# qingpingmo/OCN

Measured on AMD Instinct MI355X. Metric: candidate-edges/sec (CN predictor fwd), ogbl-collab shape, higher is better.
Workload: dtype f32

## Files before the change

### include/ocn_hip.h

```cpp
#ifndef OCN_HIP_H
#define OCN_HIP_H

#include <stdint.h>

#ifdef __cplusplus
extern "C" {
#endif

#define OCN_ABI_VERSION 9
#define OCN_EINVAL (-1)
#define OCN_ECAP   (-2)

#define OCN_ST_CAP  1
#define OCN_ST_SCAN 2
#define OCN_SCAN_POISON (-1)

#define OCN_F_CN1 1u
#define OCN_F_CN2 2u

int ocn_abi_version(void);

int64_t ocn_scan_workspace_bytes(int64_t n);

int ocn_zero_regions(void* const* ptrs, const int64_t* bytes, int32_t n, void* stream);
// ... 125 lines not shown
                          int64_t n_cols, const int64_t* rows, int64_t Q, int32_t drop_self,
                          int64_t window_cols , const int64_t* off ,
                          int64_t* edges , void* stream);
int32_t ocn_segment_topk_max_k(void);
int ocn_segment_topk(const float* scores, const int64_t* ptr, int64_t Q, int32_t k, float* top_val, int64_t* top_pos,
                     void* stream);

int ocn_philox4x32(const uint32_t* ctr , uint32_t key0, uint32_t key1, int64_t n, uint32_t* out ,
                   void* stream);
int ocn_complement_count(const int64_t* rowptrK, const int32_t* colK, int64_t n_cols, int32_t* count ,
                         void* stream);
int32_t ocn_sample_stage_cols(void);
int ocn_sample_complement_rows(const int64_t* rowptrK, const int32_t* colK, int64_t n_cols, const int64_t* rows, int64_t Q,
                               int64_t per, int64_t q0, uint64_t seed, int64_t* out , void* stream);
int ocn_sample_complement_pairs(const int64_t* rowptrK, const int32_t* colK, int64_t n_cols,
                                const int64_t* cptr , int64_t T, int64_t t0, uint64_t seed,
                                int64_t* out , void* stream);

int ocn_gather_schedule(const int32_t* gcost, int64_t n_groups, int64_t segment, int32_t* perm, void* stream);

int ocn_cn_weights_cn6(uint64_t* histA, uint64_t* histB, int64_t N, const float* innerprod, int32_t* scalars,
                       float* nip_out, const float* s2_exact , const float* s3_exact ,
                       void* stream);
int ocn_cn_gather3(const int64_t* rowptrA, const int32_t* colA, const int64_t* src, const int64_t* dst,
                   const int64_t* order, int64_t B, const int64_t* off, const uint8_t* flagsA,
                   const uint8_t* flagsB, const float* weightsA, const float* weightsB, const float* nip,
                   const float* h, int32_t H, float* xcn1, float* xcn2, float* xcn3, float* xij, void* stream);

int ocn_cn3_flags(const int64_t* rowptrA, const int32_t* colA, const int64_t* rowptrT, const int32_t* colT,
                  const uint32_t* bitmapP, int64_t bm_stride_words, const int64_t* src, const int64_t* dst,
                  const int64_t* order , int64_t B, int64_t n_cols, const int64_t* off, uint8_t* flags,
                  int64_t flags_cap, uint64_t* hist , int32_t* cnt3, int32_t* status,
                  const int64_t* nds , const int64_t* chunk_off , void* stream);

int ocn_cn_gather3_backward(const int64_t* rowptrA, const int32_t* colA, const int64_t* src, const int64_t* dst,
                            const int64_t* order, int64_t B, const int64_t* off, const uint8_t* flagsA,
                            const uint8_t* flagsB, const float* weightsA, const float* weightsB, const float* nip,
                            const float* h, int32_t H, const float* g1, const float* g2, const float* g3,
                            const float* g4, float* dh, void* stream);

int ocn_cn_gather_backward(const int64_t* rowptrA, const int32_t* colA,
                           const int64_t* src, const int64_t* dst, const int64_t* order, int64_t B,
                           const int64_t* off, const uint8_t* flags, const int32_t* wc,
                           const float* weights, const float* h, int32_t H,
                           const float* g1, const float* g2, const float* g3, float* dh, void* stream);

int64_t ocn_cn_gather_backward_det_workspace_bytes(int64_t N, int64_t B, int64_t flags_cap);
int ocn_cn_gather_backward_det(const int64_t* rowptrA, const int32_t* colA, const int64_t* src, const int64_t* dst,
                               int64_t B, const int64_t* off, const uint8_t* flags, const int32_t* wc, int64_t flags_cap,
                               const float* weights, const float* h, int64_t N, int32_t H, const float* g1,
                               const float* g2, const float* g3, float* dh, void* workspace, void* stream);
int64_t ocn_cn_gather_backward_det_keys_offset(int64_t N);
int ocn_cn_gather_backward_det_lists(const int64_t* rowptrA, const int32_t* colA, const int64_t* src, const int64_t* dst,
                                     int64_t B, const int64_t* off, const uint8_t* flags, int64_t flags_cap, int64_t N,
                                     void* workspace, void* stream);

int ocn_spmm_csr(const int64_t* rowptr, const int32_t* col, const float* val, int64_t n_rows,
                 const float* x, int32_t F, const float* pre, const float* post,
                 int32_t mode, int32_t edge_scale, int32_t self_mode,
                 float* y, void* stream);

int ocn_spmm_csr_rows(const int64_t* rowptr, const int32_t* col, const float* val, int64_t n_rows,
                      const float* x, int32_t F, const float* pre, const float* post,
                      int32_t mode, int32_t edge_scale, int32_t self_mode,
                      const int64_t* rows, int64_t n_list, float* y, void* stream);

int ocn_spmm_csr_max_arg(const int64_t* rowptr, const int32_t* col, const float* val, int64_t n_rows,
                         const float* x, int32_t F, float* y, int32_t* arg, void* stream);
int ocn_spmm_max_backward(const int64_t* rowptrT, const int32_t* colT, const float* valT, int64_t n_rows,
                          const int32_t* arg, const float* g, int32_t F, float* gx, void* stream);

int ocn_deg_rsqrt(const int64_t* rowptr, const float* val, int64_t n_rows, float add, float* out,
                  void* stream);

int64_t ocn_spgemm_max_cols(void);
int ocn_spgemm_pattern_count(const int64_t* rowptrA, const int32_t* colA, int64_t n_rows,
                             const int64_t* rowptrB, const int32_t* colB, int64_t n_colsB,
                             int32_t* row_count, uint32_t* bitmap ,
                             int64_t bm_stride_words, void* stream);
int ocn_spgemm_pattern_fill(const int64_t* rowptrA, const int32_t* colA, int64_t n_rows,
                            const int64_t* rowptrB, const int32_t* colB, int64_t n_colsB,
                            const int64_t* rowptrC, int32_t* colC, void* stream);
int32_t ocn_cn_flags_small_graph_cols(void);
int ocn_spgemm_bit_rows(const int64_t* rowptrA, const int32_t* colA, int64_t n_rows, const int64_t* rowptrB, const int32_t* colB,
                        int64_t n_colsB, const int64_t* rows, int64_t n_req, int32_t* done, uint32_t* bitmap,
                        int64_t bm_stride_words, void* stream);

int ocn_dense_from_csr(const int64_t* rowptr, const int32_t* col, int64_t n, int64_t ld, int8_t* dense, int8_t* denseT,
                       void* stream);
int ocn_dense_block_mm_bits(const int8_t* A, const int8_t* Bt, int64_t ld, int64_t K, int32_t r0, int32_t r1, int32_t c0,
                            int32_t c1, int32_t fold, uint32_t* bits, int64_t bm_stride_words, void* stream);
int ocn_bitrows_from_csr(const int64_t* rowptr, const int32_t* col, int64_t n_rows, uint32_t* bits, int64_t bm_stride_words,
                         void* stream);
int ocn_bitrows_count(const uint32_t* bits, int64_t bm_stride_words, int64_t n_rows, int64_t n_cols, int32_t* row_count,
                      void* stream);
int ocn_bitrows_fill(const uint32_t* bits, int64_t bm_stride_words, int64_t n_rows, int64_t n_cols, const int64_t* rowptr,
                     int32_t* col, void* stream);

int ocn_csr_union_count(const int64_t* rowptrA, const int32_t* colA, const int64_t* rowptrB, const int32_t* colB,
                        int64_t n_rows, int32_t* count, void* stream);
int ocn_csr_union_fill(const int64_t* rowptrA, const int32_t* colA, const int64_t* rowptrB, const int32_t* colB,
                       int64_t n_rows, const int64_t* rowptrC , int32_t* colC, void* stream);
int64_t ocn_bitrows_insert_workspace_bytes(int64_t nnzD);
int ocn_bitrows_insert(const int64_t* rowptrA, const int32_t* colA, const int64_t* rowptrT, const int32_t* colT,
                       const int64_t* rowptrD, const int32_t* colD, int64_t n, int64_t nnzD, uint32_t* bits,
                       int64_t bm_stride_words, int32_t* added, void* workspace, void* stream);

int ocn_csr_minus_count(const int64_t* rowptrA, const int32_t* colA, const int64_t* rowptrB, const int32_t* colB,
                        int64_t n_rows, int32_t* count, void* stream);
int ocn_csr_minus_fill(const int64_t* rowptrA, const int32_t* colA, const int64_t* rowptrB, const int32_t* colB,
                       int64_t n_rows, const int64_t* rowptrC , int32_t* colC, void* stream);
int64_t ocn_bitrows_remove_workspace_bytes(int64_t nnzD);
int ocn_bitrows_remove(const int64_t* rowptrA0, const int32_t* colA0, const int64_t* rowptrT0, const int32_t* colT0,
                       const int64_t* rowptrA, const int32_t* colA, const int64_t* rowptrT, const int32_t* colT,
                       const int64_t* rowptrD, const int32_t* colD, int64_t n, int64_t nnzD, uint32_t* bits,
                       int64_t bm_stride_words, int32_t* removed, void* workspace, void* stream);

int64_t ocn_rows_neighbourhood_workspace_bytes(int64_t n_list);
int ocn_rows_neighbourhood(const int64_t* rowptrT, const int32_t* colT, int64_t n, const int64_t* rows, int64_t n_list,
                           uint32_t* bits, void* workspace, void* stream);
int ocn_bitlist_count(const uint32_t* bits, int64_t n_bits, int32_t* count, void* stream);
int ocn_bitlist_fill(const uint32_t* bits, int64_t n_bits, const int64_t* off , int64_t* out,
                     void* stream);

int ocn_rows_ln_relu(const float* x, const float* gamma, const float* beta, float eps, int32_t relu,
                     int64_t rows, int32_t H, float* y, void* stream);
int ocn_combine3(const float* coef, const float* x1, const float* x2, const float* x3, int64_t n,
                 float* out, void* stream);

int ocn_fill_rows(float* dst, int64_t ld, int32_t n_cols, const float* vec, const int64_t* row_range,
                  int64_t max_rows, void* stream);

typedef struct OcnLinearGroup {
  const float* X; int64_t ldX;
  int64_t M;
  const void* Wp;
  const float* bias;
  const float* gamma; const float* beta; float eps;
  int32_t relu;
  const float* scale;
  const float* addend; int64_t ldAdd;
  const float* dotw; const float* dotb;
  float* Y; int64_t ldY;
  const int64_t* row_range;
  const int64_t* y_row_map;
  int32_t add_bcast;
} OcnLinearGroup;

int64_t ocn_linear_panel_bytes(int32_t N, int32_t K);
int ocn_linear_split_weight(const float* W, int32_t N, int32_t K, void* Wp, void* stream);
int ocn_linear_bf16x6(const float* X, int64_t M, int32_t K, const void* Wp, int32_t N,
                      const float* bias, const float* gamma, const float* beta, float eps,
                      int32_t relu, const float* dotw, const float* dotb, float* Y, void* stream);
int ocn_linear_grouped(const OcnLinearGroup* groups, int32_t n_groups, int32_t K, int32_t N, void* stream);

typedef struct OcnHeadsArgs {
  const float* x[3];
  int64_t ldx, B;
  int32_t H;
  const void* p_first[3];
  const void* p_mid[2];
  const void* p_out[3];
  const float* vec;
  const int64_t* ranges;
  const int64_t* y_row_map;
  float* y;
// ... 42 lines not shown
```

### ocn_amd/_lib.py

```python
from __future__ import annotations

import ctypes
import glob
import os
import subprocess
from ctypes import c_float, c_int32, c_int64, c_void_p

_HERE = os.path.dirname(os.path.abspath(__file__))
_ROOT = os.path.dirname(_HERE)
LIB_PATH = os.environ.get("OCN_LIB_PATH", os.path.join(_HERE, "libocn_hip.so"))
CSRC = os.path.join(_HERE, "csrc")
INCLUDE = os.path.join(_ROOT, "include")

_P = c_void_p
ABI_VERSION = 9
SIGNATURES = {
    "ocn_abi_version": (c_int32, []),
    "ocn_scan_workspace_bytes": (c_int64, [c_int64]),
    "ocn_zero_regions": (c_int32, [_P, _P, c_int32, _P]),
    "ocn_check_edges": (c_int32, [_P, _P, c_int64, c_int64, c_int64, _P, _P]),
    "ocn_edge_offsets": (c_int32, [_P, _P, c_int64, _P, _P, _P]),
    "ocn_class_order": (c_int32, [_P, _P, _P, c_int64, _P, _P, _P, _P, _P, _P]),
    "ocn_scan_i32": (c_int32, [_P, c_int64, _P, _P, _P]),
    "ocn_order_workspace_bytes": (c_int64, [c_int64]),
    "ocn_order_by_node": (c_int32, [_P, c_int64, c_int64, _P, _P, _P]),
    "ocn_order_by_node_finish": (c_int32, [_P, c_int64, c_int64, _P, _P, _P]),
    "ocn_order_by_node_finish_rec": (c_int32, [_P, _P, _P, _P, c_int64, c_int64, _P, _P, _P, _P]),
    "ocn_batch_prep": (c_int32, [_P, _P, c_int64, _P, _P, c_int64, _P, _P, _P, c_int32, _P]),
    "ocn_cn_flags": (c_int32, [_P, _P, _P, _P, _P, _P, _P, c_int64, _P, c_int64, _P, _P, _P, c_int64, c_int64, _P, _P, c_int64, _P,
                               _P, _P, _P, _P, _P, _P]),
    "ocn_cn_flags_rec": (c_int32, [_P, _P, _P, _P, _P, _P, _P, c_int64, _P, c_int64, _P, _P, _P, c_int64, c_int64, _P, _P, c_int64, _P,
                                   _P, _P, _P, _P, _P, _P]),
    "ocn_chunk_offsets": (c_int32, [_P, _P, _P, _P, c_int64, _P, _P, _P]),
    "ocn_walk_chunk": (c_int32, []),
    "ocn_cn_walk_flags": (c_int32, [_P, _P, _P, _P, _P, _P, c_int64, _P, _P, _P, c_int64, _P, _P, c_int64, _P, _P, _P,
                                    _P, _P]),
    "ocn_neighbor_degree_sum": (c_int32, [_P, _P, c_int64, _P, _P]),
    "ocn_walk_prep_max_batch": (c_int32, []),
    "ocn_cn_flags_small_graph_cols": (c_int32, []),
    "ocn_walk_prep": (c_int32, [_P, _P, _P, _P, c_int64, c_int32, _P, _P, _P, _P, _P, _P, _P, _P, _P, _P, _P, _P, _P]),
    "ocn_cn_walk_group": (c_int32, [_P, _P, _P, _P, _P, c_int64, _P, _P, _P, _P, _P, _P, _P, c_int64, _P, _P, _P, _P]),
    "ocn_walk_rev_offsets": (c_int32, [_P, _P, _P, _P, _P, c_int64, _P, _P, _P]),
    "ocn_cn_weights_cn5": (c_int32, [_P, c_int64, _P, _P, c_int32, _P, _P]),
    "ocn_cn5_column_stats": (c_int32, [_P, c_int64, _P, _P]),
    "ocn_cn_colsum_workspace_bytes": (c_int64, [c_int64, c_int64]),
    "ocn_cn_colsum_exact": (c_int32, [_P, _P, _P, c_int64, _P, _P, _P, _P, c_int64, _P, c_int64, _P, _P, _P, _P, _P, _P, _P]),
    "ocn_cn_weights_cn7": (c_int32, [_P, c_int64, c_float, _P, _P, _P]),
    "ocn_cn_gather": (c_int32, [_P, _P, _P, _P, _P, c_int64, _P, _P, _P, _P, _P, c_int32, c_int64, _P, _P, _P, _P, _P,
                                _P, _P, _P, _P, _P]),
    "ocn_cn8_pool": (c_int32, [_P, _P, _P, _P, _P, _P, _P, c_int64, _P, c_int64, _P, _P, _P, c_int64, c_int64, _P, c_int32, _P, _P,
                               _P, _P, _P, _P]),
    "ocn_cn_node_sums": (c_int32, [_P, _P, _P, _P, _P, _P, _P, c_int64, _P, c_int64, _P, _P, _P, c_int64, c_int64, _P, _P, _P, _P, _P,
                                   _P, _P]),
    "ocn_row_diff_stage_cols": (c_int32, []),
    "ocn_row_diff_count": (c_int32, [_P, _P, _P, _P, _P, c_int64, c_int32, _P, _P]),
    "ocn_row_diff_fill": (c_int32, [_P, _P, _P, _P, _P, c_int64, c_int32, _P, _P, _P]),
    "ocn_two_hop_window_cols": (c_int64, []),
    "ocn_two_hop_diff_count": (c_int32, [_P, _P, _P, _P, c_int64, _P, c_int64, c_int32, c_int64, _P, _P]),
    "ocn_two_hop_diff_fill": (c_int32, [_P, _P, _P, _P, c_int64, _P, c_int64, c_int32, c_int64, _P, _P, _P]),
    "ocn_segment_topk_max_k": (c_int32, []),
    "ocn_segment_topk": (c_int32, [_P, _P, c_int64, c_int32, _P, _P, _P]),
    "ocn_philox4x32": (c_int32, [_P, ctypes.c_uint32, ctypes.c_uint32, c_int64, _P, _P]),
    "ocn_complement_count": (c_int32, [_P, _P, c_int64, _P, _P]),
    "ocn_sample_stage_cols": (c_int32, []),
    "ocn_sample_complement_rows": (c_int32, [_P, _P, c_int64, _P, c_int64, c_int64, c_int64, ctypes.c_uint64, _P, _P]),
    "ocn_sample_complement_pairs": (c_int32, [_P, _P, c_int64, _P, c_int64, c_int64, ctypes.c_uint64, _P, _P]),
    "ocn_gather_schedule": (c_int32, [_P, c_int64, c_int64, _P, _P]),
    "ocn_coo_to_csr_workspace_bytes": (c_int64, [c_int64, c_int64, c_int32, c_int32]),
    "ocn_coo_to_csr": (c_int32, [_P, _P, c_int64, c_int64, c_int64, c_int32, c_int32, _P, _P, _P, _P, _P]),
    "ocn_wgrad_workspace_bytes": (c_int64, [c_int64, c_int32, c_int32]),
    "ocn_wgrad": (c_int32, [_P, c_int64, _P, c_int64, c_int64, c_int32, c_int32, _P, _P, _P, _P]),
    "ocn_cn_weights_cn6": (c_int32, [_P, _P, c_int64, _P, _P, _P, _P, _P, _P]),
    "ocn_cn_gather3": (c_int32, [_P, _P, _P, _P, _P, c_int64, _P, _P, _P, _P, _P, _P, _P, c_int32, _P, _P, _P, _P, _P]),
    "ocn_cn3_flags": (c_int32, [_P, _P, _P, _P, _P, c_int64, _P, _P, _P, c_int64, c_int64, _P, _P, c_int64, _P, _P, _P, _P, _P, _P]),
    "ocn_cn_gather3_backward": (c_int32, [_P, _P, _P, _P, _P, c_int64, _P, _P, _P, _P, _P, _P, _P, c_int32, _P, _P, _P, _P, _P, _P]),
    "ocn_cn_gather_backward": (c_int32, [_P, _P, _P, _P, _P, c_int64, _P, _P, _P, _P, _P, c_int32, _P, _P, _P, _P, _P]),
    "ocn_cn_gather_backward_det_workspace_bytes": (c_int64, [c_int64, c_int64, c_int64]),
    "ocn_cn_gather_backward_det": (c_int32, [_P, _P, _P, _P, c_int64, _P, _P, _P, c_int64, _P, _P, c_int64, c_int32, _P, _P, _P, _P,
                                             _P, _P]),
    "ocn_cn_gather_backward_det_keys_offset": (c_int64, [c_int64]),
    "ocn_cn_gather_backward_det_lists": (c_int32, [_P, _P, _P, _P, c_int64, _P, _P, c_int64, c_int64, _P, _P]),
    "ocn_ln_drop_relu_workspace_bytes": (c_int64, [c_int32]),
    "ocn_ln_drop_relu_forward": (c_int32, [_P, _P, _P, c_float, c_float, ctypes.c_uint64, c_int32, c_int64, c_int32, _P, _P, _P]),
    "ocn_ln_drop_relu_backward": (c_int32, [_P, _P, _P, _P, _P, c_float, ctypes.c_uint64, c_int32, c_int64, c_int32, _P, _P, _P, _P, _P]),
    "ocn_dropout_keep_mask": (c_int32, [ctypes.c_uint64, c_float, c_int64, _P, _P]),
    "ocn_mix3_workspace_bytes": (c_int64, []),
    "ocn_mix3_backward": (c_int32, [_P, _P, _P, _P, _P, c_int64, _P, _P, _P, _P, _P, _P]),
    "ocn_spmm_csr": (c_int32, [_P, _P, _P, c_int64, _P, c_int32, _P, _P, c_int32, c_int32, c_int32, _P, _P]),
    "ocn_spmm_csr_rows": (c_int32, [_P, _P, _P, c_int64, _P, c_int32, _P, _P, c_int32, c_int32, c_int32, _P, c_int64, _P, _P]),
    "ocn_spmm_csr_max_arg": (c_int32, [_P, _P, _P, c_int64, _P, c_int32, _P, _P, _P]),
    "ocn_spmm_max_backward": (c_int32, [_P, _P, _P, c_int64, _P, _P, c_int32, _P, _P]),
    "ocn_deg_rsqrt": (c_int32, [_P, _P, c_int64, c_float, _P, _P]),
    "ocn_spgemm_max_cols": (c_int64, []),
    "ocn_spgemm_pattern_count": (c_int32, [_P, _P, c_int64, _P, _P, c_int64, _P, _P, c_int64, _P]),
    "ocn_spgemm_pattern_fill": (c_int32, [_P, _P, c_int64, _P, _P, c_int64, _P, _P, _P]),
    "ocn_spgemm_bit_rows": (c_int32, [_P, _P, c_int64, _P, _P, c_int64, _P, c_int64, _P, _P, c_int64, _P]),
    "ocn_dense_from_csr": (c_int32, [_P, _P, c_int64, c_int64, _P, _P, _P]),
    "ocn_dense_block_mm_bits": (c_int32, [_P, _P, c_int64, c_int64, c_int32, c_int32, c_int32, c_int32, c_int32, _P, c_int64, _P]),
    "ocn_bitrows_from_csr": (c_int32, [_P, _P, c_int64, _P, c_int64, _P]),
    "ocn_bitrows_count": (c_int32, [_P, c_int64, c_int64, c_int64, _P, _P]),
    "ocn_bitrows_fill": (c_int32, [_P, c_int64, c_int64, c_int64, _P, _P, _P]),
    "ocn_csr_union_count": (c_int32, [_P, _P, _P, _P, c_int64, _P, _P]),
    "ocn_csr_union_fill": (c_int32, [_P, _P, _P, _P, c_int64, _P, _P, _P]),
    "ocn_bitrows_insert_workspace_bytes": (c_int64, [c_int64]),
    "ocn_bitrows_insert": (c_int32, [_P, _P, _P, _P, _P, _P, c_int64, c_int64, _P, c_int64, _P, _P, _P]),
    "ocn_csr_minus_count": (c_int32, [_P, _P, _P, _P, c_int64, _P, _P]),
    "ocn_csr_minus_fill": (c_int32, [_P, _P, _P, _P, c_int64, _P, _P, _P]),
    "ocn_bitrows_remove_workspace_bytes": (c_int64, [c_int64]),
    "ocn_bitrows_remove": (c_int32, [_P, _P, _P, _P, _P, _P, _P, _P, _P, _P, c_int64, c_int64, _P, c_int64, _P, _P, _P]),
    "ocn_rows_neighbourhood_workspace_bytes": (c_int64, [c_int64]),
    "ocn_rows_neighbourhood": (c_int32, [_P, _P, c_int64, _P, c_int64, _P, _P, _P]),
    "ocn_bitlist_count": (c_int32, [_P, c_int64, _P, _P]),
    "ocn_bitlist_fill": (c_int32, [_P, c_int64, _P, _P, _P]),
    "ocn_rows_ln_relu": (c_int32, [_P, _P, _P, c_float, c_int32, c_int64, c_int32, _P, _P]),
    "ocn_fill_rows": (c_int32, [_P, c_int64, c_int32, _P, _P, c_int64, _P]),
    "ocn_combine3": (c_int32, [_P, _P, _P, _P, c_int64, _P, _P]),
    "ocn_linear_panel_bytes": (c_int64, [c_int32, c_int32]),
    "ocn_linear_split_weight": (c_int32, [_P, c_int32, c_int32, _P, _P]),
    "ocn_linear_bf16x6": (c_int32, [_P, c_int64, c_int32, _P, c_int32, _P, _P, _P, c_float, c_int32, _P, _P,
                                    _P, _P]),
    "ocn_linear_grouped": (c_int32, [_P, c_int32, c_int32, c_int32, _P]),
    "ocn_heads_nvec": (c_int32, []),
# ... 111 lines not shown
```

### ocn_amd/csrc/cn_flags.hip

```cpp
#include "common.h"


__device__ __forceinline__ bool sampled_has(const int32_t* samp, const int32_t* __restrict__ row, i64 n,
                                            int32_t key) {
  int lo = 0, hi = OCN_WAVE;
  while (lo < hi) {
    const int mid = (lo + hi) >> 1;
    if (samp[mid] <= key) lo = mid + 1; else hi = mid;
  }
  if (lo == 0) return false;
  const int s = lo - 1;
  const i64 p0 = ((i64)s * n) >> 6, p1 = ((i64)(s + 1) * n) >> 6;
  return sorted_has(row + p0, p1 - p0, key);
}

#define T1_CAP 1024

#define LH_MAX_COLS 8192

__device__ __forceinline__ i64 wave_uniform(i64 v) {
  const unsigned lo = __builtin_amdgcn_readfirstlane((unsigned)(u64)v), hi = __builtin_amdgcn_readfirstlane((unsigned)((u64)v >> 32));
  return (i64)(((u64)hi << 32) | lo);
}
__device__ __forceinline__ bool lanes_have(int32_t t, int32_t key) {
  int pos = 0;
#pragma unroll
  for (int step = OCN_WAVE / 2; step > 0; step >>= 1)
    if (__shfl(t, pos + step - 1, OCN_WAVE) < key) pos += step;
  return __shfl(t, pos, OCN_WAVE) == key;
}

template <bool HAS_T2, bool LH, bool RECIN>
__global__ __launch_bounds__(OCN_BLOCK) void cn_flags_kernel(
    const i64* __restrict__ rowptrA, const int32_t* __restrict__ colA,
    const i64* __restrict__ rowptrT1, const int32_t* __restrict__ colT1,
    const i64* __restrict__ rowptrT2, const int32_t* __restrict__ colT2,
    const unsigned* __restrict__ bmT1, i64 bm1_stride, const unsigned* __restrict__ bmT2, i64 bm_stride,
    const i64* __restrict__ src, const i64* __restrict__ dst, const i64* __restrict__ order, i64 B,
    i64 n_cols, const i64* __restrict__ off, uint8_t* __restrict__ flags, i64 cap,
    u64* __restrict__ hist, int32_t* __restrict__ cnt1, int32_t* __restrict__ cnt2,
    int32_t* __restrict__ status, u64* rec, int32_t* __restrict__ gcost) {
  constexpr int GPB = OCN_WPB;
  __shared__ int s_cost[2][GPB];
  __shared__ int32_t s_t1[GPB][T1_CAP];
  __shared__ int32_t s_t2[GPB][OCN_WAVE];
  extern __shared__ __attribute__((aligned(16))) u64 s_hist[];
  const int gl = threadIdx.x % OCN_WAVE, g = __builtin_amdgcn_readfirstlane(threadIdx.x / OCN_WAVE);
  if (blockIdx.x == 0 && threadIdx.x == 0) status_raise(status, off[B], cap);
  const bool void_batch = off[B] < 0;
  if (LH) {
    for (i64 c = threadIdx.x; c < n_cols; c += OCN_BLOCK) s_hist[c] = 0ull;
    __syncthreads();
  }
  int par = 0;
  for (i64 e0 = (i64)blockIdx.x * GPB; e0 < B; e0 += (i64)gridDim.x * GPB, par ^= 1) {
    const i64 slot = e0 + g;
    const bool act = slot < B;
    i64 e = 0, i = 0, j = 0, a0 = 0, da = 0, b0 = 0, db = 0, c0 = 0, dc = 0, base = 0;
    const unsigned* bm_row = nullptr;
    const unsigned* bm1_row = nullptr;
    if (act) {
      if (RECIN) {
        const ulonglong2* rp = reinterpret_cast<const ulonglong2*>(rec + 4 * slot);
        const ulonglong2 ra = rp[0], rb = rp[1];
        e = wave_uniform((i64)ra.x);
        i = wave_uniform((i64)(ra.y & 0xffffffffull)); j = wave_uniform((i64)(ra.y >> 32));
        a0 = wave_uniform((i64)(rb.x & ((1ull << REC_LEN_SHIFT) - 1))); da = wave_uniform((i64)(rb.x >> REC_LEN_SHIFT));
        base = wave_uniform((i64)rb.y);
      } else {
        e = order ? order[slot] : slot;
        i = src[e]; j = dst[e];
        a0 = rowptrA[i]; da = rowptrA[i + 1] - a0;
        base = off[e];
      }
      if (bmT1) bm1_row = bmT1 + j * bm1_stride;
      else { b0 = rowptrT1[j]; db = rowptrT1[j + 1] - b0; }
      if (HAS_T2) {
        if (bmT2) bm_row = bmT2 + j * bm_stride;
        if (rowptrT2 && (LH || !bmT2)) { c0 = rowptrT2[j]; dc = rowptrT2[j + 1] - c0; }
      }
      if (void_batch) { da = 0; db = 0; dc = 0; base = 0; }
    }
    const bool t1_reg = db <= OCN_WAVE, t1_lds = db <= T1_CAP;
    int32_t t1 = 0x7fffffff;
    if (t1_reg) { if (gl < db) t1 = colT1[b0 + gl]; }
    else if (t1_lds)
      for (i64 q = gl; q < db; q += OCN_WAVE) s_t1[g][q] = colT1[b0 + q];
    const bool t2_full = HAS_T2 && rowptrT2 && dc == n_cols;
    if (HAS_T2 && !t2_full && !bmT2) {
      if (dc > OCN_WAVE) s_t2[g][gl] = colT2[c0 + (((i64)gl * dc) >> 6)];
      else if (gl < dc) s_t2[g][gl] = colT2[c0 + gl];
    }
    wave_lds_sync();
    const bool fits = base + da <= cap;
    int c1 = 0, c2 = 0;
    for (i64 p0 = 0; p0 < da; p0 += OCN_WAVE) {
      const i64 p = p0 + gl;
      const bool in = p < da;
      const int32_t k = in ? colA[a0 + p] : 0;
      unsigned w2 = 0;
      if (HAS_T2 && bmT2 && !t2_full && in) w2 = bm_row[k >> 5];
      bool f1;
      if (bmT1) f1 = in && ((bm1_row[k >> 5] >> (k & 31)) & 1u);
      else if (t1_reg) f1 = lanes_have(t1, k) && in;
      else f1 = in && (t1_lds ? sorted_has(&s_t1[g][0], db, k) : sorted_has(colT1 + b0, db, k));
      bool f2 = false;
      if (HAS_T2 && in) {
        if (t2_full) f2 = true;
        else if (bmT2) f2 = (w2 >> (k & 31)) & 1u;
        else f2 = dc > OCN_WAVE ? sampled_has(&s_t2[g][0], colT2 + c0, dc, k) : sorted_has(&s_t2[g][0], dc, k);
      }
      if (fits && in) flags[base + p] = (uint8_t)((f1 ? OCN_F_CN1 : 0u) | (f2 ? OCN_F_CN2 : 0u));
      if (f1 | f2) {
        const u64 inc = (u64)f1 | ((u64)f2 << HF_BITS) | (1ull << (2 * HF_BITS));
        if (LH) atomicAdd(s_hist + k, inc); else atomicAdd(hist + 2 * (i64)k, inc);
      }
      c1 += f1;
      c2 += f2;
    }
    wave_lds_sync();
#pragma unroll
    for (int o = OCN_WAVE / 2; o > 0; o >>= 1) {
      c1 += __shfl_xor(c1, o, OCN_WAVE);
      c2 += __shfl_xor(c2, o, OCN_WAVE);
    }
    if (act && gl == 0) {
      cnt1[e] = c1;
      if (cnt2) cnt2[e] = c2;
      if (rec) {
        u64* r = rec + 4 * slot;
        if (!RECIN) {
          r[0] = (u64)e;
          r[1] = (u64)i | ((u64)j << 32);
        }
        if (!RECIN || void_batch) r[2] = (u64)a0 | ((u64)da << REC_LEN_SHIFT);
        r[3] = (u64)base | ((u64)(da > 0 && (i64)c2 == da) << REC_FULL2_BIT) | ((u64)(c1 > 0) << 62) | ((u64)(c2 > 0) << 63);
      }
    }
    if (gcost) {
      if (gl == 0) s_cost[par][g] = act ? c1 + c2 : 0;
      __syncthreads();
      if (threadIdx.x == 0) {
        int t = 0;
#pragma unroll
        for (int q = 0; q < GPB; ++q) t = SCHED_COST(t, s_cost[par][q]);
        gcost[e0 / GPB] = t;
      }
    }
  }
  if (LH) {
    __syncthreads();
    for (i64 c = threadIdx.x; c < n_cols; c += OCN_BLOCK) {
      const u64 v = s_hist[c];
      if (v) atomicAdd(hist + 2 * c, v);
    }
  }
}

extern "C" {

int32_t ocn_cn_flags_small_graph_cols(void) { return LH_MAX_COLS; }

static int cn_flags_launch(const int64_t* rowptrA, const int32_t* colA, const int64_t* rowptrT1,
                           const int32_t* colT1, const int64_t* rowptrT2, const int32_t* colT2,
                           const uint32_t* bitmapT1, int64_t bm1_stride_words, const uint32_t* bitmapT2, int64_t bm_stride_words,
                           const int64_t* src, const int64_t* dst, const int64_t* order, int64_t B,
                           int64_t n_cols, const int64_t* off, uint8_t* flags, int64_t flags_cap, uint64_t* hist,
                           int32_t* cnt1, int32_t* cnt2, int32_t* status, uint64_t* rec, int32_t* gcost, bool rec_in, void* stream) {
  if (B < 0 || flags_cap < 0 || B > (int64_t)HF_MASK) return OCN_EINVAL;
  if (B == 0) return 0;
  if (!rowptrA || (!rowptrT1 && !bitmapT1) || !src || !dst || !off || !hist || !cnt1 || !status) return OCN_EINVAL;
  if (rec_in && (!rec || !order)) return OCN_EINVAL;
  if ((bitmapT1 && bm1_stride_words * 32 < n_cols) || (bitmapT2 && bm_stride_words * 32 < n_cols)) return OCN_EINVAL;
  constexpr int GPB = OCN_WPB;
  hipStream_t st = (hipStream_t)stream;
  const bool lh = n_cols > 0 && n_cols <= LH_MAX_COLS;
  const size_t lds = lh ? (size_t)n_cols * sizeof(u64) : 0;
  const int grid = lh ? grid_for((B + GPB - 1) / GPB, 256 * 3) : grid_for((B + GPB - 1) / GPB);
  if (lh) {
    static bool raised_dev[64] = {};
    int devid = 0;
    if (hipGetDevice(&devid) != hipSuccess || devid < 0 || devid >= 64) return OCN_EINVAL;
    bool& raised = raised_dev[devid];
    if (!raised) {
      const void* fns[4] = {(const void*)cn_flags_kernel<true, true, false>, (const void*)cn_flags_kernel<false, true, false>,
                            (const void*)cn_flags_kernel<true, true, true>, (const void*)cn_flags_kernel<false, true, true>};
      for (const void* fn : fns) {
        hipError_t e1 = hipFuncSetAttribute(fn, hipFuncAttributeMaxDynamicSharedMemorySize, LH_MAX_COLS * (int)sizeof(u64));
        if (e1 != hipSuccess) return (int)e1;
      }
      raised = true;
    }
  }
#define CN_FLAGS_ARGS(T2P, T2C)                                                                      \
  (const i64*)rowptrA, colA, (const i64*)rowptrT1, colT1, (const i64*)(T2P), (T2C),                   \
      (const unsigned*)bitmapT1, (i64)bm1_stride_words, (const unsigned*)bitmapT2, (i64)bm_stride_words, (const i64*)src, \
      (const i64*)dst, (const i64*)order, (i64)B, (i64)n_cols, (const i64*)off, flags, (i64)flags_cap, \
      (u64*)hist, cnt1, cnt2, status, (u64*)rec, gcost
#define CN_FLAGS_LAUNCH(T2, LHV, RI, T2P, T2C)                                                        \
  hipLaunchKernelGGL((cn_flags_kernel<T2, LHV, RI>), dim3(grid), dim3(OCN_BLOCK), (LHV) ? lds : 0, st, CN_FLAGS_ARGS(T2P, T2C))
#define CN_FLAGS_PICK(T2, T2P, T2C)                                                                   \
  do {                                                                                                \
    if (lh) { if (rec_in) CN_FLAGS_LAUNCH(T2, true, true, T2P, T2C); else CN_FLAGS_LAUNCH(T2, true, false, T2P, T2C); }   \
    else { if (rec_in) CN_FLAGS_LAUNCH(T2, false, true, T2P, T2C); else CN_FLAGS_LAUNCH(T2, false, false, T2P, T2C); }    \
  } while (0)
  if (!rowptrT2 && bitmapT2 && lh) return OCN_EINVAL;
  if (rowptrT2 || bitmapT2) CN_FLAGS_PICK(true, rowptrT2, colT2);
  else CN_FLAGS_PICK(false, nullptr, (const int32_t*)nullptr);
#undef CN_FLAGS_PICK
#undef CN_FLAGS_LAUNCH
  return launch_status();
}

int ocn_cn_flags(const int64_t* rowptrA, const int32_t* colA, const int64_t* rowptrT1,
                 const int32_t* colT1, const int64_t* rowptrT2, const int32_t* colT2,
                 const uint32_t* bitmapT1, int64_t bm1_stride_words, const uint32_t* bitmapT2, int64_t bm_stride_words,
                 const int64_t* src, const int64_t* dst, const int64_t* order, int64_t B,
                 int64_t n_cols, const int64_t* off, uint8_t* flags, int64_t flags_cap, uint64_t* hist,
                 int32_t* cnt1, int32_t* cnt2, int32_t* status, uint64_t* rec, int32_t* gcost, void* stream) {
  return cn_flags_launch(rowptrA, colA, rowptrT1, colT1, rowptrT2, colT2, bitmapT1, bm1_stride_words, bitmapT2, bm_stride_words,
                         src, dst, order, B, n_cols, off, flags, flags_cap, hist, cnt1, cnt2, status, rec, gcost, false, stream);
}

int ocn_cn_flags_rec(const int64_t* rowptrA, const int32_t* colA, const int64_t* rowptrT1,
                     const int32_t* colT1, const int64_t* rowptrT2, const int32_t* colT2,
                     const uint32_t* bitmapT1, int64_t bm1_stride_words, const uint32_t* bitmapT2, int64_t bm_stride_words,
                     const int64_t* src, const int64_t* dst, const int64_t* order, int64_t B,
                     int64_t n_cols, const int64_t* off, uint8_t* flags, int64_t flags_cap, uint64_t* hist,
                     int32_t* cnt1, int32_t* cnt2, int32_t* status, uint64_t* rec, int32_t* gcost, void* stream) {
  return cn_flags_launch(rowptrA, colA, rowptrT1, colT1, rowptrT2, colT2, bitmapT1, bm1_stride_words, bitmapT2, bm_stride_words,
                         src, dst, order, B, n_cols, off, flags, flags_cap, hist, cnt1, cnt2, status, rec, gcost, true, stream);
}

}
```

### ocn_amd/ops.py

```python
from __future__ import annotations

import ctypes
import os
from typing import Optional, Tuple

import torch
from torch import Tensor

from . import _lib
from ._lib import check, ptr, stream_ptr

FLAGS_NOSYNC_LIMIT = 1 << 30
validate_indices = True
stage_timer = None
LN_WIDTHS = (16, 32, 64, 128, 256, 512)
a1_bitmap_max_bytes = int(os.environ.get("OCN_A1_BITMAP_MAX_BYTES", 64 << 20))
a2_bitmap_max_bytes = 16 << 30
skip_zero_rows = True
skip_zero_min_share = 0.15
skip_zero_backoff = 32
skip_zero_min_batch = 4096
walk_two_sided = True
walk_share_min = 2
sort_edges_min_batch = 4096
# ... 1297 lines not shown
    return out


@_on_device
def mix3_backward(coef: Tensor, g: Tensor, x1: Tensor, x2: Tensor, x3: Tensor):
    g = _req(g.contiguous(), torch.float32, "g")
    for t, nm in ((x1, "x1"), (x2, "x2"), (x3, "x3")):
        if _req(t, torch.float32, nm).shape != g.shape:
            raise ValueError("mix3_backward: shape mismatch")
    n = g.numel()
    if n % 4:
        raise ValueError("mix3_backward: n must be a multiple of 4")
    l = _lib.lib()
    d1, d2, d3 = torch.empty_like(g), torch.empty_like(g), torch.empty_like(g)
    dcoef = torch.empty(3, dtype=torch.float32, device=g.device)
    ws = torch.empty(int(l.ocn_mix3_workspace_bytes()), dtype=torch.uint8, device=g.device)
    check(l.ocn_mix3_backward(ptr(coef), ptr(g), ptr(x1), ptr(x2), ptr(x3), n, ptr(d1), ptr(d2), ptr(d3), ptr(dcoef), ptr(ws),
                              stream_ptr()), "ocn_mix3_backward")
    return d1, d2, d3, dcoef


@_on_device
def fill_rows(dst: Tensor, vec: Tensor, row_range: Tensor) -> None:
    _req_strided(dst, "dst")
    _req(vec, torch.float32, "vec")
    _req(row_range, torch.int64, "row_range", 1)
    if vec.numel() != dst.shape[1]:
        raise ValueError("fill_rows: width mismatch")
    check(_lib.lib().ocn_fill_rows(ptr(dst), dst.stride(0), dst.shape[1], ptr(vec), ptr(row_range), dst.shape[0],
                                   stream_ptr()), "ocn_fill_rows")
    _mark("mlp_glue")


LINEAR_WIDTHS = (32, 64, 128, 256)
fast_linear = True
_panels: dict = {}


@_on_device
def linear_panel(weight: Tensor) -> Tensor:
    import weakref
    key = id(weight)
    hit = _panels.get(key)
    if (hit is not None and hit[0]() is weight and hit[1] == weight.data_ptr() and hit[2] == weight._version
            and hit[3] == tuple(weight.shape)):
        return hit[4]
    w = _req(weight.detach(), torch.float32, "weight", 2)
    N, K = w.shape
    panel = torch.empty(int(_lib.lib().ocn_linear_panel_bytes(N, K)), dtype=torch.uint8, device=w.device)
    check(_lib.lib().ocn_linear_split_weight(ptr(w), N, K, ptr(panel), stream_ptr()), "ocn_linear_split_weight")
    if len(_panels) > 512:
        for k in [k for k, v in _panels.items() if v[0]() is None]:
            del _panels[k]
    _panels[key] = (weakref.ref(weight), weight.data_ptr(), weight._version, (N, K), panel)
    return panel


@_on_device
def heads_panel(weight: Tensor):
    import math
    w = _req(weight.detach(), torch.float32, "weight", 2)
    N, K = w.shape
    m = float(w.abs().max().item()) if w.numel() else 0.0
    if not math.isfinite(m):
        raise ValueError("heads_panel: non-finite weight")
    sw = 13 - math.frexp(m)[1] + 1 if m > 0.0 else 0
    sw = max(-100, min(100, sw))
    panel = torch.empty(int(_lib.lib().ocn_heads_panel_bytes(N, K)), dtype=torch.uint8, device=w.device)
    check(_lib.lib().ocn_heads_split_weight(ptr(w), N, K, float(2.0 ** sw), ptr(panel), stream_ptr()), "ocn_heads_split_weight")
    return panel, float(2.0 ** -sw)


HEADS_WIDTHS = (128, 256)
train_linear = True
train_tails = os.environ.get("OCN_TRAIN_TAILS", "1") != "0"
fused_heads = True
fused_heads_min_width = 128


def heads_small_batch(max_rows: int = -1) -> int:
    return int(_lib.lib().ocn_heads_small_batch(int(max_rows)))


@_on_device
def heads_fused(x1: Tensor, x2: Tensor, xij: Tensor, pack: dict, ranges: Optional[Tensor], y_row_map: Optional[Tensor],
                b_on_union: bool, scratch: Tensor, dump: Optional[Tensor] = None) -> Optional[Tensor]:
    for t, nm in ((x1, "xcn1"), (x2, "xcn2"), (xij, "xij")):
        _req(t, torch.float32, nm, 2)
    B, H = xij.shape
    if x1.shape != (B, H) or x2.shape != (B, H) or H not in HEADS_WIDTHS:
        raise ValueError("heads_fused: shape mismatch")
    a = _lib.OcnHeadsArgs()
    a.x[0], a.x[1], a.x[2] = x1.data_ptr(), x2.data_ptr(), xij.data_ptr()
    a.ldx, a.B, a.H = H, B, H
    for i in range(3):
        a.p_first[i] = pack["first"][i].data_ptr()
        a.p_out[i] = pack["out"][i].data_ptr()
    a.p_mid[0], a.p_mid[1] = pack["mid"][0].data_ptr(), pack["mid"][1].data_ptr()
    a.vec = pack["vec"].data_ptr()
    a.ranges = 0 if ranges is None else _req(ranges, torch.int64, "ranges").data_ptr()
    a.y_row_map = 0 if y_row_map is None else _req(y_row_map, torch.int64, "y_row_map", 1).data_ptr()
    y = None
    nconst = int(_lib.lib().ocn_heads_const_bytes(H)) // 4
    if dump is None:
        y = torch.empty((B, 1), dtype=torch.float32, device=xij.device)
        a.y = y.data_ptr()
        if _req(pack["cpark"], torch.float32, "cpark", 1).numel() != nconst:
            raise ValueError("heads_fused: constants buffer of the wrong size")
        a.cpark = pack["cpark"].data_ptr()
    else:
        if B != 1 or _req(dump, torch.float32, "dump", 1).numel() != nconst:
            raise ValueError("heads_fused: constants mode takes one row and ocn_heads_const_bytes(H) bytes")
        a.dump = dump.data_ptr()
    if scratch.numel() * scratch.element_size() < int(_lib.lib().ocn_heads_scratch_bytes(H)):
        raise ValueError("heads_fused: scratch too small")
    a.scratch = scratch.data_ptr()
    a.eps, a.ln, a.b_on_union = float(pack["eps"]), int(pack["ln"]), int(bool(b_on_union))
    _mark("mlp_glue")
    check(_lib.lib().ocn_heads_fused(ctypes.byref(a), stream_ptr()), "ocn_heads_fused")
    _mark("linear", pack["flops_per_row"] * B)
    return y


def linear_ok(x: Tensor, weight: Tensor) -> bool:
    return (fast_linear and x.is_cuda and x.dim() == 2 and x.dtype == torch.float32 and x.is_contiguous()
            and weight.shape[0] in LINEAR_WIDTHS and weight.shape[1] % 16 == 0 and weight.shape[1] == x.shape[1])


@_on_device
def linear(x: Tensor, weight: Tensor, bias: Optional[Tensor] = None, ln=None, relu: bool = False,
           dot=None, y_row_map: Optional[Tensor] = None) -> Tensor:
    _req(x, torch.float32, "x", 2)
    M, K = x.shape
    N = weight.shape[0]
    if y_row_map is not None:
        if dot is None:
            raise ValueError("y_row_map needs the dot epilogue")
        y = torch.empty((M, 1), dtype=torch.float32, device=x.device)
        linear_grouped([dict(x=x, weight=weight, bias=bias, ln=ln, relu=relu, dot=(dot[0].reshape(1, -1), dot[1]), y=y,
                             y_row_map=y_row_map)], K, N)
        return y
    panel = linear_panel(weight)
    _mark("mlp_glue")
    y = torch.empty((M, 1) if dot is not None else (M, N), dtype=torch.float32, device=x.device)
    g = b = None
    eps = 0.0
    if ln is not None:
        g, b, eps = ln
    dw = db = None
    if dot is not None:
        dw, db = dot
        dw = dw.reshape(-1)
    check(_lib.lib().ocn_linear_bf16x6(ptr(x), M, K, ptr(panel), N, ptr(bias), ptr(g), ptr(b), float(eps),
                                       int(relu), ptr(dw), ptr(db), ptr(y), stream_ptr()), "ocn_linear_bf16x6")
    _mark("linear", 2.0 * M * K * N)
    return y


def linear_ok_t(gy: Tensor, weight: Tensor) -> bool:
    return (fast_linear and gy.is_cuda and gy.dim() == 2 and gy.dtype == torch.float32
            and weight.shape[1] in LINEAR_WIDTHS and weight.shape[0] % 16 == 0 and weight.shape[0] == gy.shape[1])


@_on_device
def linear_t(gy: Tensor, weight: Tensor) -> Tensor:
    gy = _req(gy.contiguous(), torch.float32, "gy", 2)
# ... 112 lines not shown
```

Measured before the change: 171.4 million.

## Process two candidate edges per wave in cn_flags kernel for large batches

Adds an NS template parameter so each wave handles two edge slots at once on large graphs when the batch is big enough. The two slots split the shared-memory T1/T2 staging, share the colA load and fold their histogram atomics into one when the source node matches, and read packed records through a single lane load plus readlane. The aim is fewer per-edge wave iterations and less wave-serial latency on short adjacency rows, at the cost of more registers, extra control flow and possible imbalance when the two rows differ in length. gcost output is regrouped per SCHED_GROUP to stay consistent.

```diff
diff --git a/include/ocn_hip.h b/include/ocn_hip.h
--- a/include/ocn_hip.h
+++ b/include/ocn_hip.h
@@ -231,6 +231,7 @@
                             const int64_t* rowptrB, const int32_t* colB, int64_t n_colsB,
                             const int64_t* rowptrC, int32_t* colC, void* stream);
 int32_t ocn_cn_flags_small_graph_cols(void);
+int64_t ocn_cn_flags_pair_min_batch(int64_t min_rows);
 int ocn_spgemm_bit_rows(const int64_t* rowptrA, const int32_t* colA, int64_t n_rows, const int64_t* rowptrB, const int32_t* colB,
                         int64_t n_colsB, const int64_t* rows, int64_t n_req, int32_t* done, uint32_t* bitmap,
                         int64_t bm_stride_words, void* stream);
diff --git a/ocn_amd/_lib.py b/ocn_amd/_lib.py
--- a/ocn_amd/_lib.py
+++ b/ocn_amd/_lib.py
@@ -38,6 +38,7 @@
     "ocn_neighbor_degree_sum": (c_int32, [_P, _P, c_int64, _P, _P]),
     "ocn_walk_prep_max_batch": (c_int32, []),
     "ocn_cn_flags_small_graph_cols": (c_int32, []),
+    "ocn_cn_flags_pair_min_batch": (c_int64, [c_int64]),
     "ocn_walk_prep": (c_int32, [_P, _P, _P, _P, c_int64, c_int32, _P, _P, _P, _P, _P, _P, _P, _P, _P, _P, _P, _P, _P]),
     "ocn_cn_walk_group": (c_int32, [_P, _P, _P, _P, _P, c_int64, _P, _P, _P, _P, _P, _P, _P, c_int64, _P, _P, _P, _P]),
     "ocn_walk_rev_offsets": (c_int32, [_P, _P, _P, _P, _P, c_int64, _P, _P, _P]),
diff --git a/ocn_amd/csrc/cn_flags.hip b/ocn_amd/csrc/cn_flags.hip
--- a/ocn_amd/csrc/cn_flags.hip
+++ b/ocn_amd/csrc/cn_flags.hip
@@ -30,7 +30,7 @@
   return __shfl(t, pos, OCN_WAVE) == key;
 }
 
-template <bool HAS_T2, bool LH, bool RECIN>
+template <bool HAS_T2, bool LH, bool RECIN, int NS>
 __global__ __launch_bounds__(OCN_BLOCK) void cn_flags_kernel(
     const i64* __restrict__ rowptrA, const int32_t* __restrict__ colA,
     const i64* __restrict__ rowptrT1, const int32_t* __restrict__ colT1,
@@ -40,7 +40,9 @@
     i64 n_cols, const i64* __restrict__ off, uint8_t* __restrict__ flags, i64 cap,
     u64* __restrict__ hist, int32_t* __restrict__ cnt1, int32_t* __restrict__ cnt2,
     int32_t* __restrict__ status, u64* rec, int32_t* __restrict__ gcost) {
-  constexpr int GPB = OCN_WPB;
+  constexpr int GPB = OCN_WPB, SPB = GPB * NS;
+  constexpr int T1_PART = T1_CAP / NS, T2_PART = OCN_WAVE / NS;
+  static_assert(NS == 1 || (NS == 2 && !LH), "slot pairs: large-graph forms only");
   __shared__ int s_cost[2][GPB];
   __shared__ int32_t s_t1[GPB][T1_CAP];
   __shared__ int32_t s_t2[GPB][OCN_WAVE];
@@ -53,98 +55,174 @@
     __syncthreads();
   }
   int par = 0;
-  for (i64 e0 = (i64)blockIdx.x * GPB; e0 < B; e0 += (i64)gridDim.x * GPB, par ^= 1) {
-    const i64 slot = e0 + g;
-    const bool act = slot < B;
-    i64 e = 0, i = 0, j = 0, a0 = 0, da = 0, b0 = 0, db = 0, c0 = 0, dc = 0, base = 0;
-    const unsigned* bm_row = nullptr;
-    const unsigned* bm1_row = nullptr;
-    if (act) {
-      if (RECIN) {
-        const ulonglong2* rp = reinterpret_cast<const ulonglong2*>(rec + 4 * slot);
-        const ulonglong2 ra = rp[0], rb = rp[1];
-        e = wave_uniform((i64)ra.x);
-        i = wave_uniform((i64)(ra.y & 0xffffffffull)); j = wave_uniform((i64)(ra.y >> 32));
-        a0 = wave_uniform((i64)(rb.x & ((1ull << REC_LEN_SHIFT) - 1))); da = wave_uniform((i64)(rb.x >> REC_LEN_SHIFT));
-        base = wave_uniform((i64)rb.y);
+  for (i64 e0 = (i64)blockIdx.x * SPB; e0 < B; e0 += (i64)gridDim.x * SPB, par ^= 1) {
+    i64 slot[NS];
+    bool act[NS];
+    i64 e[NS], i[NS], j[NS], a0[NS], da[NS], b0[NS], db[NS], c0[NS], dc[NS], base[NS];
+    const unsigned* bm_row[NS];
+    const unsigned* bm1_row[NS];
+#pragma unroll
+    for (int s = 0; s < NS; ++s) {
+      slot[s] = e0 + NS * g + s;
+      act[s] = slot[s] < B;
+      e[s] = i[s] = j[s] = a0[s] = da[s] = b0[s] = db[s] = c0[s] = dc[s] = base[s] = 0;
+      bm_row[s] = bm1_row[s] = nullptr;
+    }
+    u64 recw = 0;
+    if (RECIN && NS > 1 && gl < 4 * NS && slot[0] + gl / 4 < B) recw = rec[4 * slot[0] + gl];
+#pragma unroll
+    for (int s = 0; s < NS; ++s)
+      if (act[s]) {
+        if (RECIN) {
+          u64 w[4];
+          if (NS == 1) {
+            const ulonglong2* rp = reinterpret_cast<const ulonglong2*>(rec + 4 * slot[s]);
+            const ulonglong2 ra = rp[0], rb = rp[1];
+            w[0] = ra.x; w[1] = ra.y; w[2] = rb.x; w[3] = rb.y;
+          } else {
+#pragma unroll
+            for (int q = 0; q < 4; ++q)
+              w[q] = (u64)(unsigned)__builtin_amdgcn_readlane((int)(unsigned)recw, 4 * s + q) |
+                     ((u64)(unsigned)__builtin_amdgcn_readlane((int)(unsigned)(recw >> 32), 4 * s + q) << 32);
+          }
+          e[s] = wave_uniform((i64)w[0]);
+          i[s] = wave_uniform((i64)(w[1] & 0xffffffffull)); j[s] = wave_uniform((i64)(w[1] >> 32));
+          a0[s] = wave_uniform((i64)(w[2] & ((1ull << REC_LEN_SHIFT) - 1))); da[s] = wave_uniform((i64)(w[2] >> REC_LEN_SHIFT));
+          base[s] = wave_uniform((i64)w[3]);
+        } else {
+          e[s] = order ? order[slot[s]] : slot[s];
+          i[s] = src[e[s]]; j[s] = dst[e[s]];
+          a0[s] = rowptrA[i[s]]; da[s] = rowptrA[i[s] + 1] - a0[s];
+          base[s] = off[e[s]];
+        }
+        if (bmT1) bm1_row[s] = bmT1 + j[s] * bm1_stride;
+        else { b0[s] = rowptrT1[j[s]]; db[s] = rowptrT1[j[s] + 1] - b0[s]; }
+        if (HAS_T2) {
+          if (bmT2) bm_row[s] = bmT2 + j[s] * bm_stride;
+          if (rowptrT2 && (LH || !bmT2)) { c0[s] = rowptrT2[j[s]]; dc[s] = rowptrT2[j[s] + 1] - c0[s]; }
+        }
+        if (void_batch) { da[s] = 0; db[s] = 0; dc[s] = 0; base[s] = 0; }
+      }
+    bool t1_reg[NS], t1_lds[NS], t2_full[NS], t2_lds[NS];
+    int t1_at[NS], t2_at[NS];
+    int32_t t1[NS];
+#pragma unroll
+    for (int s = 0; s < NS; ++s) {
+      const int o = (s + 1) % NS;
+      const bool whole1 = NS == 1 || db[o] <= OCN_WAVE;
+      t1_reg[s] = db[s] <= OCN_WAVE; t1_lds[s] = db[s] <= (whole1 ? T1_CAP : T1_PART);
+      t1_at[s] = whole1 ? 0 : s * T1_PART;
+      t1[s] = 0x7fffffff;
+      if (t1_reg[s]) { if (gl < db[s]) t1[s] = colT1[b0[s] + gl]; }
+      else if (t1_lds[s])
+        for (i64 q = gl; q < db[s]; q += OCN_WAVE) s_t1[g][t1_at[s] + q] = colT1[b0[s] + q];
+    }
+#pragma unroll
+    for (int s = 0; s < NS; ++s) {
+      const int o = (s + 1) % NS;
+      t2_full[s] = HAS_T2 && rowptrT2 && dc[s] == n_cols;
+      const bool whole2 = NS == 1 || (HAS_T2 && rowptrT2 && dc[o] == n_cols) || dc[o] == 0;
+      t2_lds[s] = whole2 || dc[s] <= T2_PART;
+      t2_at[s] = whole2 ? 0 : s * T2_PART;
+      if (HAS_T2 && !t2_full[s] && !bmT2 && t2_lds[s]) {
+        if (dc[s] > OCN_WAVE) s_t2[g][gl] = colT2[c0[s] + (((i64)gl * dc[s]) >> 6)];
+        else if (gl < dc[s]) s_t2[g][t2_at[s] + gl] = colT2[c0[s] + gl];
+      }
+    }
+    wave_lds_sync();
+    bool fits[NS];
+    int c1[NS], c2[NS];
+    i64 da_max = da[0];
+#pragma unroll
+    for (int s = 0; s < NS; ++s) {
+      fits[s] = base[s] + da[s] <= cap;
+      c1[s] = c2[s] = 0;
+      if (s > 0 && da[s] > da_max) da_max = da[s];
+    }
+    const bool same = NS > 1 && i[0] == i[NS - 1];
+    for (i64 p0 = 0; p0 < da_max; p0 += OCN_WAVE) {
+      const i64 p = p0 + gl;
+      bool in[NS], f1[NS], f2[NS];
+      int32_t k[NS];
+      unsigned w2[NS];
+#pragma unroll
+      for (int s = 0; s < NS; ++s) {
+        in[s] = p < da[s];
+        if (s > 0 && same) k[s] = k[0];
+        else k[s] = in[s] ? colA[a0[s] + p] : 0;
+      }
+#pragma unroll
+      for (int s = 0; s < NS; ++s) {
+        w2[s] = 0;
+        if (HAS_T2 && bmT2 && !t2_full[s] && in[s]) w2[s] = bm_row[s][k[s] >> 5];
+      }
+#pragma unroll
+      for (int s = 0; s < NS; ++s) {
+        if (bmT1) f1[s] = in[s] && ((bm1_row[s][k[s] >> 5] >> (k[s] & 31)) & 1u);
+        else if (t1_reg[s]) f1[s] = lanes_have(t1[s], k[s]) && in[s];
+        else f1[s] = in[s] && (t1_lds[s] ? sorted_has(&s_t1[g][t1_at[s]], db[s], k[s]) : sorted_has(colT1 + b0[s], db[s], k[s]));
+      }
+#pragma unroll
+      for (int s = 0; s < NS; ++s) {
+        f2[s] = false;
+        if (HAS_T2 && in[s]) {
+          if (t2_full[s]) f2[s] = true;
+          else if (bmT2) f2[s] = (w2[s] >> (k[s] & 31)) & 1u;
+          else if (!t2_lds[s]) f2[s] = sorted_has(colT2 + c0[s], dc[s], k[s]);
+          else f2[s] = dc[s] > OCN_WAVE ? sampled_has(&s_t2[g][0], colT2 + c0[s], dc[s], k[s]) : sorted_has(&s_t2[g][t2_at[s]], dc[s], k[s]);
+        }
+        if (fits[s] && in[s]) flags[base[s] + p] = (uint8_t)((f1[s] ? OCN_F_CN1 : 0u) | (f2[s] ? OCN_F_CN2 : 0u));
+      }
+      if (NS > 1 && same) {
+        u64 inc = 0;
+#pragma unroll
+        for (int s = 0; s < NS; ++s) inc += (u64)f1[s] | ((u64)f2[s] << HF_BITS) | ((u64)(f1[s] | f2[s]) << (2 * HF_BITS));
+        if (inc) atomicAdd(hist + 2 * (i64)k[0], inc);
       } else {
-        e = order ? order[slot] : slot;
-        i = src[e]; j = dst[e];
-        a0 = rowptrA[i]; da = rowptrA[i + 1] - a0;
-        base = off[e];
-      }
-      if (bmT1) bm1_row = bmT1 + j * bm1_stride;
-      else { b0 = rowptrT1[j]; db = rowptrT1[j + 1] - b0; }
-      if (HAS_T2) {
-        if (bmT2) bm_row = bmT2 + j * bm_stride;
-        if (rowptrT2 && (LH || !bmT2)) { c0 = rowptrT2[j]; dc = rowptrT2[j + 1] - c0; }
-      }
-      if (void_batch) { da = 0; db = 0; dc = 0; base = 0; }
-    }
-    const bool t1_reg = db <= OCN_WAVE, t1_lds = db <= T1_CAP;
-    int32_t t1 = 0x7fffffff;
-    if (t1_reg) { if (gl < db) t1 = colT1[b0 + gl]; }
-    else if (t1_lds)
-      for (i64 q = gl; q < db; q += OCN_WAVE) s_t1[g][q] = colT1[b0 + q];
-    const bool t2_full = HAS_T2 && rowptrT2 && dc == n_cols;
-    if (HAS_T2 && !t2_full && !bmT2) {
-      if (dc > OCN_WAVE) s_t2[g][gl] = colT2[c0 + (((i64)gl * dc) >> 6)];
-      else if (gl < dc) s_t2[g][gl] = colT2[c0 + gl];
+#pragma unroll
+        for (int s = 0; s < NS; ++s)
+          if (f1[s] | f2[s]) {
+            const u64 inc = (u64)f1[s] | ((u64)f2[s] << HF_BITS) | (1ull << (2 * HF_BITS));
+            if (LH) atomicAdd(s_hist + k[s], inc); else atomicAdd(hist + 2 * (i64)k[s], inc);
+          }
+      }
+#pragma unroll
+      for (int s = 0; s < NS; ++s) {
+        c1[s] += __popcll(__ballot(f1[s]));
+        c2[s] += __popcll(__ballot(f2[s]));
+      }
     }
     wave_lds_sync();
-    const bool fits = base + da <= cap;
-    int c1 = 0, c2 = 0;
-    for (i64 p0 = 0; p0 < da; p0 += OCN_WAVE) {
-      const i64 p = p0 + gl;
-      const bool in = p < da;
-      const int32_t k = in ? colA[a0 + p] : 0;
-      unsigned w2 = 0;
-      if (HAS_T2 && bmT2 && !t2_full && in) w2 = bm_row[k >> 5];
-      bool f1;
-      if (bmT1) f1 = in && ((bm1_row[k >> 5] >> (k & 31)) & 1u);
-      else if (t1_reg) f1 = lanes_have(t1, k) && in;
-      else f1 = in && (t1_lds ? sorted_has(&s_t1[g][0], db, k) : sorted_has(colT1 + b0, db, k));
-      bool f2 = false;
-      if (HAS_T2 && in) {
-        if (t2_full) f2 = true;
-        else if (bmT2) f2 = (w2 >> (k & 31)) & 1u;
-        else f2 = dc > OCN_WAVE ? sampled_has(&s_t2[g][0], colT2 + c0, dc, k) : sorted_has(&s_t2[g][0], dc, k);
-      }
-      if (fits && in) flags[base + p] = (uint8_t)((f1 ? OCN_F_CN1 : 0u) | (f2 ? OCN_F_CN2 : 0u));
-      if (f1 | f2) {
-        const u64 inc = (u64)f1 | ((u64)f2 << HF_BITS) | (1ull << (2 * HF_BITS));
-        if (LH) atomicAdd(s_hist + k, inc); else atomicAdd(hist + 2 * (i64)k, inc);
-      }
-      c1 += f1;
-      c2 += f2;
-    }
-    wave_lds_sync();
-#pragma unroll
-    for (int o = OCN_WAVE / 2; o > 0; o >>= 1) {
-      c1 += __shfl_xor(c1, o, OCN_WAVE);
-      c2 += __shfl_xor(c2, o, OCN_WAVE);
-    }
-    if (act && gl == 0) {
-      cnt1[e] = c1;
-      if (cnt2) cnt2[e] = c2;
-      if (rec) {
-        u64* r = rec + 4 * slot;
-        if (!RECIN) {
-          r[0] = (u64)e;
-          r[1] = (u64)i | ((u64)j << 32);
+#pragma unroll
+    for (int s = 0; s < NS; ++s)
+      if (act[s] && gl == 0) {
+        cnt1[e[s]] = c1[s];
+        if (cnt2) cnt2[e[s]] = c2[s];
+        if (rec) {
+          u64* r = rec + 4 * slot[s];
+          if (!RECIN) {
+            r[0] = (u64)e[s];
+            r[1] = (u64)i[s] | ((u64)j[s] << 32);
+          }
+          if (!RECIN || void_batch) r[2] = (u64)a0[s] | ((u64)da[s] << REC_LEN_SHIFT);
+          r[3] = (u64)base[s] | ((u64)(da[s] > 0 && (i64)c2[s] == da[s]) << REC_FULL2_BIT) | ((u64)(c1[s] > 0) << 62) | ((u64)(c2[s] > 0) << 63);
         }
-        if (!RECIN || void_batch) r[2] = (u64)a0 | ((u64)da << REC_LEN_SHIFT);
-        r[3] = (u64)base | ((u64)(da > 0 && (i64)c2 == da) << REC_FULL2_BIT) | ((u64)(c1 > 0) << 62) | ((u64)(c2 > 0) << 63);
-      }
-    }
+      }
     if (gcost) {
-      if (gl == 0) s_cost[par][g] = act ? c1 + c2 : 0;
+      int cost = act[0] ? c1[0] + c2[0] : 0;
+#pragma unroll
+      for (int s = 1; s < NS; ++s) cost = SCHED_COST(cost, act[s] ? c1[s] + c2[s] : 0);
+      if (gl == 0) s_cost[par][g] = cost;
       __syncthreads();
       if (threadIdx.x == 0) {
-        int t = 0;
-#pragma unroll
-        for (int q = 0; q < GPB; ++q) t = SCHED_COST(t, s_cost[par][q]);
-        gcost[e0 / GPB] = t;
+#pragma unroll
+        for (int q = 0; q < NS; ++q)
+          if (NS == 1 || e0 + q * SCHED_GROUP < B) {
+            int t = 0;
+#pragma unroll
+            for (int w = 0; w < GPB / NS; ++w) t = SCHED_COST(t, s_cost[par][q * (GPB / NS) + w]);
+            gcost[e0 / SCHED_GROUP + q] = t;
+          }
       }
     }
   }
@@ -160,6 +238,14 @@
 extern "C" {
 
 int32_t ocn_cn_flags_small_graph_cols(void) { return LH_MAX_COLS; }
+
+static int64_t g_flags_pair_min_batch = 32768;
+
+int64_t ocn_cn_flags_pair_min_batch(int64_t min_rows) {
+  const int64_t prev = g_flags_pair_min_batch;
+  if (min_rows >= 0) g_flags_pair_min_batch = min_rows;
+  return prev;
+}
 
 static int cn_flags_launch(const int64_t* rowptrA, const int32_t* colA, const int64_t* rowptrT1,
                            const int32_t* colT1, const int64_t* rowptrT2, const int32_t* colT2,
@@ -176,15 +262,17 @@
   hipStream_t st = (hipStream_t)stream;
   const bool lh = n_cols > 0 && n_cols <= LH_MAX_COLS;
   const size_t lds = lh ? (size_t)n_cols * sizeof(u64) : 0;
-  const int grid = lh ? grid_for((B + GPB - 1) / GPB, 256 * 3) : grid_for((B + GPB - 1) / GPB);
+  const bool pairs = !lh && B >= g_flags_pair_min_batch;
+  const int spb = pairs ? 2 * GPB : GPB;
+  const int grid = lh ? grid_for((B + GPB - 1) / GPB, 256 * 3) : grid_for((B + spb - 1) / spb);
   if (lh) {
     static bool raised_dev[64] = {};
     int devid = 0;
     if (hipGetDevice(&devid) != hipSuccess || devid < 0 || devid >= 64) return OCN_EINVAL;
     bool& raised = raised_dev[devid];
     if (!raised) {
-      const void* fns[4] = {(const void*)cn_flags_kernel<true, true, false>, (const void*)cn_flags_kernel<false, true, false>,
-                            (const void*)cn_flags_kernel<true, true, true>, (const void*)cn_flags_kernel<false, true, true>};
+      const void* fns[4] = {(const void*)cn_flags_kernel<true, true, false, 1>, (const void*)cn_flags_kernel<false, true, false, 1>,
+                            (const void*)cn_flags_kernel<true, true, true, 1>, (const void*)cn_flags_kernel<false, true, true, 1>};
       for (const void* fn : fns) {
         hipError_t e1 = hipFuncSetAttribute(fn, hipFuncAttributeMaxDynamicSharedMemorySize, LH_MAX_COLS * (int)sizeof(u64));
         if (e1 != hipSuccess) return (int)e1;
@@ -197,12 +285,13 @@
       (const unsigned*)bitmapT1, (i64)bm1_stride_words, (const unsigned*)bitmapT2, (i64)bm_stride_words, (const i64*)src, \
       (const i64*)dst, (const i64*)order, (i64)B, (i64)n_cols, (const i64*)off, flags, (i64)flags_cap, \
       (u64*)hist, cnt1, cnt2, status, (u64*)rec, gcost
-#define CN_FLAGS_LAUNCH(T2, LHV, RI, T2P, T2C)                                                        \
-  hipLaunchKernelGGL((cn_flags_kernel<T2, LHV, RI>), dim3(grid), dim3(OCN_BLOCK), (LHV) ? lds : 0, st, CN_FLAGS_ARGS(T2P, T2C))
+#define CN_FLAGS_LAUNCH(T2, LHV, RI, NSV, T2P, T2C)                                                   \
+  hipLaunchKernelGGL((cn_flags_kernel<T2, LHV, RI, NSV>), dim3(grid), dim3(OCN_BLOCK), (LHV) ? lds : 0, st, CN_FLAGS_ARGS(T2P, T2C))
 #define CN_FLAGS_PICK(T2, T2P, T2C)                                                                   \
   do {                                                                                                \
-    if (lh) { if (rec_in) CN_FLAGS_LAUNCH(T2, true, true, T2P, T2C); else CN_FLAGS_LAUNCH(T2, true, false, T2P, T2C); }   \
-    else { if (rec_in) CN_FLAGS_LAUNCH(T2, false, true, T2P, T2C); else CN_FLAGS_LAUNCH(T2, false, false, T2P, T2C); }    \
+    if (lh) { if (rec_in) CN_FLAGS_LAUNCH(T2, true, true, 1, T2P, T2C); else CN_FLAGS_LAUNCH(T2, true, false, 1, T2P, T2C); }   \
+    else if (pairs) { if (rec_in) CN_FLAGS_LAUNCH(T2, false, true, 2, T2P, T2C); else CN_FLAGS_LAUNCH(T2, false, false, 2, T2P, T2C); }   \
+    else { if (rec_in) CN_FLAGS_LAUNCH(T2, false, true, 1, T2P, T2C); else CN_FLAGS_LAUNCH(T2, false, false, 1, T2P, T2C); }    \
   } while (0)
   if (!rowptrT2 && bitmapT2 && lh) return OCN_EINVAL;
   if (rowptrT2 || bitmapT2) CN_FLAGS_PICK(true, rowptrT2, colT2);
diff --git a/ocn_amd/ops.py b/ocn_amd/ops.py
--- a/ocn_amd/ops.py
+++ b/ocn_amd/ops.py
@@ -1403,6 +1403,10 @@
     return int(_lib.lib().ocn_heads_small_batch(int(max_rows)))
 
 
+def flags_pair_min_batch(min_rows: int = -1) -> int:
+    return int(_lib.lib().ocn_cn_flags_pair_min_batch(int(min_rows)))
+
+
 @_on_device
 def heads_fused(x1: Tensor, x2: Tensor, xij: Tensor, pack: dict, ranges: Optional[Tensor], y_row_map: Optional[Tensor],
                 b_on_union: bool, scratch: Tensor, dump: Optional[Tensor] = None) -> Optional[Tensor]:
```

Result: faster. 177.8 million, median of 6 (+3.8%).
